# CHONSPQX/modulated-deform-conv

Hardware: AMD Instinct MI355X
Metric: fwd+bwd GSamples/s, MDCN2d 3x3 C=256 56x56 B=32; %HBM roofline (higher is better)
Workload: dtype f32; 1 GPU; ModulatedDeformConv2d 3x3, C_in=C_out=256, 56x56, deformable_group=1, fp32, B=32 per GPU, forward+backward (BASELINE.json configs[1]); global_batch=32, parallelism=dp1 batch-sharded

## Files before the change

### include/mdconv.h

```cpp
#ifndef MDCONV_H_
#define MDCONV_H_

#include <stddef.h>

#ifdef __cplusplus
extern "C" {
#endif

#define MDCONV_ABI_VERSION 2
#define MDCONV_DESC_V2 0x100

enum { MDCONV_F32 = 0, MDCONV_F16 = 1, MDCONV_F64 = 2, MDCONV_BF16 = 3 };
#define MDCONV_SAMPLING_F32 0x10
#define MDCONV_WGRAD_F32 0x40

enum {
  MDCONV_OK = 0,
  MDCONV_EINVAL = -1,
  MDCONV_ENULL = -2,
  MDCONV_EWORKSPACE = -3,
  MDCONV_ELAUNCH = -4,
  MDCONV_EUNSUPPORTED = -5
};

// ... 32 lines not shown

#define MDCONV_DESC_INIT(nd) { (nd) | MDCONV_DESC_V2, 0, 0, 0, 0, 0, {0, 0, 1}, {0, 0, 1}, {1, 1, 1}, \
                               {0, 0, 0}, {1, 1, 1}, 1, 1, 64, 0, 1, 0, 0, {0, 0, 0, 0, 0} }

int mdconv_abi_version(void);
const char *mdconv_last_error(void);

int mdconv_out_size(const mdconv_desc *d, int axis);

size_t mdconv_workspace_bytes(const mdconv_desc *d, int backward);

int mdconv_set_path(int path);
int mdconv_last_path(void);
enum { MDCONV_KERNELS_DIRECT = 1, MDCONV_KERNELS_F32 = 2, MDCONV_KERNELS_HP = 3, MDCONV_KERNELS_DEPTHWISE = 4 };
int mdconv_last_kernels(void);
int mdconv_planned_kernels(const mdconv_desc *d, int backward);

int mdconv_profile_enable(int on);
int mdconv_profile_read(int which, double *total_ms);
const char *mdconv_profile_name(int which);
void mdconv_profile_reset(void);

int mdconv_set_accumulate(int on);

enum { MDCONV_LAYOUT_NCHW = 0, MDCONV_LAYOUT_CHANNELS_LAST = 1 };
int mdconv_set_input_layout(int layout);
int mdconv_input_layout_supported(const mdconv_desc *d, int layout, int backward);

int mdconv_result_layout_supported(const mdconv_desc *d, int backward);

// ... 198 lines not shown
```

### modulated_deform_conv_amd/_capi.py

```python
import ctypes
import os
import threading

HERE = os.path.dirname(os.path.abspath(__file__))
LIB_PATH = os.environ.get("MDCONV_LIB") or os.path.join(HERE, "libmdconv_hip.so")

F32, F16, F64, BF16 = 0, 1, 2, 3
SAMPLING_F32 = 0x10
WGRAD_F32 = 0x40
PATH_AUTO, PATH_DIRECT, PATH_MFMA, PATH_DEPTHWISE = 0, 1, 2, 3
ABI_VERSION = 2
DESC_V2 = 0x100
FLAG_DETERMINISTIC = 1
FLAG_NO_GRAD_INPUT = 4
FLAG_NO_GRAD_WEIGHT = 8
FLAG_MATH_BF16 = 32
FLAG_OUTPUT_CHANNELS_LAST = 64
FLAG_GRAD_INPUT_CHANNELS_LAST = 128
FLAG_SOFTMAX = 256

EXPORTS = (
    "mdconv_abi_version", "mdconv_last_error", "mdconv_out_size", "mdconv_workspace_bytes",
    "mdconv_set_path", "mdconv_last_path", "mdconv_last_kernels",
    "mdconv_profile_enable", "mdconv_profile_read", "mdconv_profile_reset", "mdconv_profile_name",
    "mdconv_stream_wait_weight_ready", "mdconv_stream_wait_weight_ready_on", "mdconv_set_accumulate", "mdconv_set_input_layout",
    "mdconv_input_layout_supported", "mdconv_deterministic_supported", "mdconv_math_bf16_used",
    "mdconv_result_layout_supported", "mdconv_planned_kernels",
    "mdconv_deform_conv2d_forward", "mdconv_deform_conv2d_backward",
    "mdconv_modulated_deform_conv2d_forward", "mdconv_modulated_deform_conv2d_backward",
    "mdconv_deform_conv3d_forward", "mdconv_deform_conv3d_backward",
    "mdconv_modulated_deform_conv3d_forward", "mdconv_modulated_deform_conv3d_backward",
    "mdconv_dcnv3_out_size", "mdconv_dcnv3_workspace_bytes", "mdconv_dcnv3_forward", "mdconv_dcnv3_backward",
    "mdconv_msda_value_len", "mdconv_msda_workspace_bytes", "mdconv_msda_forward", "mdconv_msda_backward",
    "mdconv_dcnv4_out_size", "mdconv_dcnv4_offset_mask_len", "mdconv_dcnv4_workspace_bytes", "mdconv_dcnv4_forward",
    "mdconv_dcnv4_backward",
    "mdconv_fda_value_len", "mdconv_fda_loc_attn_len", "mdconv_fda_workspace_bytes", "mdconv_fda_forward", "mdconv_fda_backward",
    "mdconv_droi_workspace_bytes", "mdconv_droi_forward", "mdconv_droi_backward",
    "mdconv_msda3d_value_len", "mdconv_msda3d_workspace_bytes", "mdconv_msda3d_forward", "mdconv_msda3d_backward",
)

EXPORTS_DAGG = ("mdconv_dagg_feature_len", "mdconv_dagg_workspace_bytes", "mdconv_dagg_forward", "mdconv_dagg_backward")
EXPORTS_MSDAP = ("mdconv_msdap_value_len", "mdconv_msdap_points_len", "mdconv_msdap_workspace_bytes", "mdconv_msdap_forward",
                 "mdconv_msdap_backward")
EXPORTS_FDAP = ("mdconv_fdap_value_len", "mdconv_fdap_loc_attn_len", "mdconv_fdap_workspace_bytes", "mdconv_fdap_forward",
                "mdconv_fdap_backward")
EXPORTS_AFDA = ("mdconv_afda_value_len", "mdconv_afda_offs_attn_len", "mdconv_afda_workspace_bytes", "mdconv_afda_forward",
                "mdconv_afda_backward")

SAMP_QUERIES = {"dcnv3": ("out_size",), "msda": ("value_len",), "dcnv4": ("out_size", "offset_mask_len"),
                "fda": ("value_len", "loc_attn_len"), "droi": (), "msda3d": ("value_len",), "dagg": ("feature_len",),
                "msdap": ("value_len", "points_len"), "fdap": ("value_len", "loc_attn_len"),
                "afda": ("value_len", "offs_attn_len")}

# ... 113 lines not shown
        L.mdconv_last_kernels.restype = ctypes.c_int
        L.mdconv_input_layout_supported.argtypes = [ctypes.c_void_p, ctypes.c_int, ctypes.c_int]
        L.mdconv_deterministic_supported.restype = ctypes.c_int
        L.mdconv_deterministic_supported.argtypes = [ctypes.c_void_p, ctypes.c_int]
        has_math_query = hasattr(L, "mdconv_math_bf16_used")
        if has_math_query:
            L.mdconv_math_bf16_used.argtypes = [ctypes.c_void_p, ctypes.c_int]
        has_layout_query = hasattr(L, "mdconv_result_layout_supported")
        if has_layout_query:
            L.mdconv_result_layout_supported.argtypes = [ctypes.c_void_p, ctypes.c_int]
        has_plan_query = hasattr(L, "mdconv_planned_kernels")
        if has_plan_query:
            L.mdconv_planned_kernels.argtypes = [ctypes.c_void_p, ctypes.c_int]
        missing = (() if has_math_query else ("mdconv_math_bf16_used",)) + (() if has_layout_query else ("mdconv_result_layout_supported",))
        missing += () if has_plan_query else ("mdconv_planned_kernels",)
        missing += tuple(n for n in EXPORTS + EXPORTS_DAGG + EXPORTS_MSDAP + EXPORTS_FDAP + EXPORTS_AFDA
                         if n.startswith(tuple("mdconv_%s_" % op for op in SAMP_QUERIES)) and not hasattr(L, n))
        for name in EXPORTS[11:] + EXPORTS_DAGG + EXPORTS_MSDAP + EXPORTS_FDAP + EXPORTS_AFDA:
            if name not in missing:
                getattr(L, name).restype = ctypes.c_int
        for op, queries in SAMP_QUERIES.items():
            if not hasattr(L, "mdconv_%s_workspace_bytes" % op):
                continue
            ws = getattr(L, "mdconv_%s_workspace_bytes" % op)
            ws.restype, ws.argtypes = ctypes.c_size_t, [ctypes.c_void_p, ctypes.c_int]
            for q in queries:
                getattr(L, "mdconv_%s_%s" % (op, q)).argtypes = [ctypes.c_void_p] + ([ctypes.c_int] if q == "out_size" else [])
        if L.mdconv_abi_version() != ABI_VERSION:
            raise ImportError("libmdconv_hip.so ABI version mismatch")
        _lib = L
# ... 25 lines not shown
    prev = lib().mdconv_set_path(names[path] if isinstance(path, str) else int(path))
    return {v: k for k, v in names.items()}[prev]


def last_path():
    return {0: "none", PATH_DIRECT: "direct", PATH_MFMA: "mfma", PATH_DEPTHWISE: "depthwise"}[lib().mdconv_last_path()]


def last_kernels():
    return KERNELS[lib().mdconv_last_kernels()]


KERNELS = {0: "none", 1: "direct", 2: "f32", 3: "hp", 4: "depthwise"}


def planned_kernels(desc, backward):
    return KERNELS[lib().mdconv_planned_kernels(ctypes.byref(desc), int(bool(backward)))]


PROFILE_SLOTS = 5


_modes = threading.local()


def accumulate_mode():
    return getattr(_modes, "accumulate", 1)


class overwrite_grads:
# ... 156 lines not shown
```

### modulated_deform_conv_amd/csrc/mdconv_api.hip

```cpp
#include <stdarg.h>
#include <stdio.h>
#include <stdlib.h>
#include <string.h>

#include <atomic>
#include <iterator>
#include <map>
#include <mutex>
#include <utility>

#include "mdconv_common.hpp"
#include "dw_plan.hpp"
#include "hp_plan.hpp"
#include "mfma_plan.hpp"
#include "samp_api.hpp"

namespace mdconv {

static thread_local char g_err[512] = "";
static thread_local int g_last_path = 0;
static thread_local int g_last_kernels = 0;
static thread_local int g_accumulate = 1;
static thread_local int g_input_layout = 0;
static std::mutex g_wready_mu;
struct WReady { hipEvent_t ev; unsigned long long tick; };
static std::map<std::pair<int, hipStream_t>, WReady> g_wready;
static std::map<int, hipEvent_t> g_wready_latest;
static unsigned long long g_wready_tick = 0;
constexpr size_t kWReadyMax = 64;
static std::atomic<int> g_path{-1};

void set_error(const char *fmt, ...) {
  va_list ap;
  va_start(ap, fmt);
  vsnprintf(g_err, sizeof(g_err), fmt, ap);
  va_end(ap);
// ... 335 lines not shown

static int refuse(const CallPlan &cp, const Geom &g, int dt, int path, bool backward) {
  if (cp.refused == REFUSE_CHANNELS_LAST)
    set_error("channels-last input is only supported by the native 16-bit kernels with C_in a multiple of 32");
  else if (cp.refused == REFUSE_PATH_MFMA)
    set_error("MDCONV_PATH=mfma but this shape/dtype is not supported by the MFMA kernels");
  else if (cp.refused == REFUSE_RESULT_LAYOUT)
    set_layout_refusal(cp, backward);
  else if (cp.refused == REFUSE_PATH_DEPTHWISE)
    set_error("MDCONV_PATH=depthwise but the depthwise kernels do not take this call: %s", cp.dw_reason);
  else
    set_det_refusal(g, dt, path);
  return MDCONV_EUNSUPPORTED;
}

static int run_forward(const mdconv_desc *d, int nd, int modulated, Tensors t, void *ws,
                       size_t ws_bytes, void *stream) {
  g_err[0] = 0;
  Geom g;
  int rc = fill_geom(d, &g);
  if (rc) return rc;
  if (g.nd != nd || (d->modulated != 0) != (modulated != 0)) {
    set_error("descriptor (ndim=%d, modulated=%d) does not match this entry point", g.nd,
              d->modulated);
    return MDCONV_EINVAL;
  }
  Modes md;
  if ((rc = call_modes(d, &md))) return rc;
  if ((rc = require(t.input, "input")) || (rc = require(t.weight, "weight")) ||
      (rc = require(t.offset, "offset")) || (rc = require(t.output, "output")))
    return rc;
  if (modulated && (rc = require(t.mask, "mask"))) return rc;
  if (g.with_bias && (rc = require(t.bias, "bias"))) return rc;
// ... 36 lines not shown
      if (cp.route == ROUTE_F32_SAMP32) return samp32_forward(g, dt, cp.s32, t, ws, s);
      return mfma_forward(g, dt, cp.f32, t, ws, s);
    default:
      g_last_path = MDCONV_PATH_DIRECT;
      g_last_kernels = MDCONV_KERNELS_DIRECT;
      note_direct_fallback(g, dt, false, path);
      if (cp.route != ROUTE_DIRECT_SAMP32) return direct_forward(g, dt, t, s);
      if ((rc = check_ws(ws, ws_bytes, cp.bytes))) return rc;
      return samp32_forward(g, dt, cp.s32, t, ws, s);
  }
}

static int run_backward(const mdconv_desc *d, int nd, int modulated, Tensors t, void *ws,
                        size_t ws_bytes, void *stream) {
  g_err[0] = 0;
  Geom g;
  int rc = fill_geom(d, &g);
  if (rc) return rc;
  if (g.nd != nd || (d->modulated != 0) != (modulated != 0)) {
    set_error("descriptor (ndim=%d, modulated=%d) does not match this entry point", g.nd,
              d->modulated);
    return MDCONV_EINVAL;
  }
  Modes md;
  if ((rc = call_modes(d, &md))) return rc;
  const Skip skip = md.skip;
  if (skip.input) t.grad_input = nullptr;
  if (skip.weight) t.grad_weight = t.grad_bias = nullptr;
  if ((rc = require(t.input, "input")) || (rc = require(t.weight, "weight")) ||
      (rc = require(t.offset, "offset")) || (rc = require(t.grad_output, "grad_output")) ||
// ... 249 lines not shown
int mdconv_stream_wait_weight_ready(void *stream) {
  return wait_weight_ready((hipStream_t)stream, false, nullptr);
}

int mdconv_stream_wait_weight_ready_on(void *stream, void *producer_stream) {
  return wait_weight_ready((hipStream_t)stream, true, (hipStream_t)producer_stream);
}

int mdconv_set_path(int path) {
  const int prev = current_path();
  if (path >= MDCONV_PATH_AUTO && path <= MDCONV_PATH_DEPTHWISE) g_path.store(path);
  return prev;
}
int mdconv_last_path(void) { return g_last_path; }
int mdconv_last_kernels(void) { return g_last_kernels; }

int mdconv_deform_conv2d_forward(const mdconv_desc *d, const void *input, const void *weight,
                                 const void *bias, const void *offset, void *output,
                                 void *workspace, size_t workspace_bytes, void *stream) {
  Tensors t = {};
  t.input = input; t.weight = weight; t.bias = bias; t.offset = offset; t.output = output;
  return run_forward(d, 2, 0, t, workspace, workspace_bytes, stream);
}

int mdconv_deform_conv2d_backward(const mdconv_desc *d, const void *input, const void *weight,
                                  const void *bias, const void *offset, void *grad_input,
                                  void *grad_weight, void *grad_bias, void *grad_offset,
                                  const void *grad_output, void *workspace,
                                  size_t workspace_bytes, void *stream) {
  Tensors t = {};
// ... 76 lines not shown
```

### modulated_deform_conv_amd/csrc/mdconv_common.hpp

```cpp
#pragma once
#include <hip/hip_runtime.h>
#include <hip/hip_fp16.h>
#include <stdint.h>
#include <functional>

#include "../../include/mdconv.h"

namespace mdconv {

#define MDCONV_EPS 1.192092896e-07F

struct Geom {
  int nd, B, C, O, G, DG, K;
  int in_sz[3], out_sz[3], ksz[3], stride[3], pad[3], dil[3];
  int S_i, S_o;
  int Cg, Og, Cdg;
  int N;
  int load_eps;
  int atom_eps;
  int range_gate;
  int with_bias;
  int modulated;
  int acc_data, acc_w;
  int in_cl;
  int cm_pad, cm_real, C_caller;
  int det;
};
__host__ __device__ __forceinline__ int caller_channel(const Geom &g, int c) {
  if (g.cm_pad == 0) return c < g.C ? c : -1;
  const int q = c / g.cm_pad, r = c - q * g.cm_pad;
  return (q < g.DG && r < g.cm_real) ? q * g.cm_real + r : -1;
}
__host__ __device__ __forceinline__ int caller_channels(const Geom &g) { return g.cm_pad ? g.C_caller : g.C; }

template <typename T> struct Acc { using type = float; };
template <> struct Acc<double> { using type = double; };

__device__ __forceinline__ float ld(const float *p) { return *p; }
__device__ __forceinline__ double ld(const double *p) { return *p; }
__device__ __forceinline__ float ld(const __half *p) { return __half2float(*p); }
__device__ __forceinline__ void st(float *p, float v) { *p = v; }
__device__ __forceinline__ void st(double *p, double v) { *p = v; }
__device__ __forceinline__ void st(__half *p, float v) { *p = __float2half(v); }
struct bf16_t { unsigned short bits; };
__device__ __forceinline__ float bf16_bits_to_float(unsigned short b) { return __uint_as_float((unsigned)b << 16); }
__device__ __forceinline__ unsigned short float_to_bf16_bits(float v) {
  const unsigned u = __float_as_uint(v);
  if ((u & 0x7fffffffu) > 0x7f800000u) return (unsigned short)((u >> 16) | 0x40u);
// ... 345 lines not shown
```

### modulated_deform_conv_amd/csrc/mfma_bwd_data.hip

```cpp
#include "mfma_kernels.hpp"
#include "mfma_tile.hpp"
#include <algorithm>
#include <map>
#include <mutex>
#include <stdio.h>
#include <stdlib.h>

namespace mdconv {

namespace {

int grid_for(int64_t total) {
  int64_t b = (total + 255) / 256;
  return (int)(b > 8192 ? 8192 : (b < 1 ? 1 : b));
}

__device__ __forceinline__ void pack_wq_items(const Geom &g, int ochunks, int cblks, const float *__restrict__ w,
                                              float *__restrict__ wq, int64_t first, int64_t step) {
  const int64_t total = (int64_t)g.K * ochunks * cblks * 2 * 64;
  for (int64_t i = first; i < total; i += step) {
    int64_t r = i;
    const int lane = (int)(r & 63); r >>= 6;
    const int q = (int)(r & 1); r >>= 1;
    const int cblk = (int)(r % cblks); r /= cblks;
// ... 28 lines not shown
    pack_wq_items(g, ochunks, cblks, w, wq, (int64_t)bid * 256 + threadIdx.x, (int64_t)nb_pack * 256);
    return;
  }
  bid -= nb_pack;
  if (bid < nb_zero) {
    for (int64_t i = (int64_t)bid * 256 + threadIdx.x; i < cnt_n; i += (int64_t)nb_zero * 256) cnt[i] = 0;
    return;
  }
  bid -= nb_zero;
  const int qx = bid % qtiles, cy = (bid / qtiles) % ctiles, b = bid / (qtiles * ctiles);
  nchw_to_nhwc_tile(t, g.C, g.S_i, x, xt, b, cy * 32, qx * 32);
}



template <int ND, bool MOD, int WAVES_C, int QPQ, bool CL>
__global__ __launch_bounds__(256, 2) void mfma_bwd_data_kernel(
    Geom g, BwdDims bd, const float *__restrict__ input, const float *__restrict__ gout,
    const float *__restrict__ wq, const float *__restrict__ offset, const float *__restrict__ mask,
    float *__restrict__ gcol, float *__restrict__ grad_offset, float *__restrict__ grad_mask,
    float *__restrict__ ga, float *__restrict__ bias_part, int *__restrict__ cnt,
    int *__restrict__ table, const float *__restrict__ xt, int ntiles, int n_full, int n_tail, int tpw) {
  constexpr int NC = 1 << ND, NP = NC / 2;
  constexpr int MB = 2;
  constexpr int WAVES_P = 4 / WAVES_C;
  constexpr int BNP = 32 * WAVES_P;
  constexpr int RB = ND == 2 ? 8 : 4;
  constexpr int NBATCH = MB * 16 / RB;
  constexpr int HS = NBATCH / 2, CPS = NC / HS;
  constexpr int kOob = 0x7ffffff0;
  extern __shared__ __attribute__((aligned(16))) float smem[];
  const int T_o = bd.ochunks;
  const int gpitch = T_o * 16 + 4;
  float *Gs = smem;
  float *red = smem + BNP * gpitch;
  const int kTapGroup = bd.tap_group;

  const int tid = threadIdx.x, lane = tid & 63, kh = lane >> 5;
  const int wave = __builtin_amdgcn_readfirstlane(tid >> 6);
  const int wc = wave / WAVES_P, wp = wave % WAVES_P;

  int u0, u1;
  if ((int)blockIdx.x < n_full) {
    u0 = xcd_remap(blockIdx.x, n_full) * g.K * tpw;
    u1 = u0 + g.K * tpw;
// ... 717 lines not shown
  }
  return n;
}

size_t bwd_data_lds_bytes(const Geom &g, const BwdDims &bd) {
  const int bnp = 32 * (4 / bd.waves_c);
  const int passes = bd.cblks_q / (2 * bd.waves_c);
  const size_t red = (size_t)bd.red_floats;
  const size_t cl = bd.cl_drain ? (size_t)4 * 32 * 64 + (size_t)4 * 32 * (2 * (1 << g.nd) + 4) : 0;
  return ((size_t)bnp * (bd.ochunks * 16 + 4) + red + cl) * sizeof(float);
}

int mfma_bwd_data_f32(const Geom &g, const BwdDims &bd, const Tensors &t, const float *wq,
                      float *gcol, float *ga, float *bias_part, int *cnt, int *table,
                      const float *xt, hipStream_t stream) {
#define LAUNCH_BD_(ND, MOD, WC, QPQ, CL)                                                            \
  do {                                                                                          \
    const int bnp = 32 * (4 / WC);                                                              \
    const int ntiles = (g.N + bnp - 1) / bnp;                                                   \
    const size_t lds = bwd_data_lds_bytes(g, bd);                                               \
     \
     \
     \
     \
    static std::once_flag attr_once;                                                            \
    static hipError_t attr_err = hipSuccess;                                                    \
    std::call_once(attr_once, [] {                                                              \
      attr_err = hipFuncSetAttribute((const void *)mfma_bwd_data_kernel<ND, MOD, WC, QPQ, CL>,  \
                                     hipFuncAttributeMaxDynamicSharedMemorySize, (int)kBwdDataLdsCap); \
    });                                                                                         \
    if (attr_err != hipSuccess) { set_error("hipFuncSetAttribute: %s", hipGetErrorString(attr_err)); return MDCONV_ELAUNCH; } \
     \
     \
    int occ_q = 0;                                                                              \
    {                                                                                           \
      static std::mutex occ_mu;                                                                 \
      static std::map<size_t, int> occ_by_lds;                                                  \
      std::lock_guard<std::mutex> lock(occ_mu);                                                 \
      auto it = occ_by_lds.find(lds);                                                           \
      if (it == occ_by_lds.end()) {                                                             \
        int nq = 0;                                                                             \
        (void)hipOccupancyMaxActiveBlocksPerMultiprocessor(                                     \
            &nq, (const void *)mfma_bwd_data_kernel<ND, MOD, WC, QPQ, CL>, 256, lds);           \
        (void)hipGetLastError();                                                                \
        it = occ_by_lds.emplace(lds, nq > 0 ? nq : (lds * 2 <= 160 * 1024 ? 2 : 1)).first;      \
      }                                                                                         \
      occ_q = it->second;                                                                       \
    }                                                                                           \
    const int slots = num_cus() * occ_q;                                                        \
    const int tpw = 2;                        \
    const int n_full = ntiles / (slots * tpw) * slots;                                          \
    static const bool debug_plan = getenv("MDCONV_DEBUG_PLAN") != nullptr;                      \
    if (debug_plan)                                                                             \
      fprintf(stderr, "[mdconv] GEMM-1 plan: %d tiles, %zu B LDS, %d resident per CU\n", ntiles, lds, occ_q); \
    const int n_tail = (int)std::min<int64_t>((int64_t)(ntiles - n_full * tpw) * g.K, slots);   \
    hipLaunchKernelGGL((mfma_bwd_data_kernel<ND, MOD, WC, QPQ, CL>), dim3(n_full + n_tail), \
                       dim3(256), lds, stream,                                                  \
                       g, bd, (const float *)t.input, (const float *)t.grad_output, wq,         \
                       (const float *)t.offset, (const float *)t.mask, gcol,                    \
                       (float *)t.grad_offset, (float *)t.grad_mask, ga, bias_part, cnt, table, xt,        \
                       ntiles, n_full, n_tail, tpw);                                            \
  } while (0)
                                                \
#define LAUNCH_BD(ND, MOD, WC, QPQ)                                                             \
  do {                                                                                          \
    if (xt != nullptr && bd.cl_drain) LAUNCH_BD_(ND, MOD, WC, QPQ, true);                       \
    else LAUNCH_BD_(ND, MOD, WC, QPQ, false);                                                   \
  } while (0)
#define LAUNCH_BD2(ND, MOD)                                                                     \
  do {                                                                                          \
    const int nbatch = ND == 2 ? 4 : 8, nquads = bd.ochunks / 4;                                \
                   \
    const int qpq = (ND == 2 && g.G == 1 && nquads % nbatch == 0 && nquads / nbatch <= 2) ? nquads / nbatch : 0; \
    if (bd.waves_c == 4) {                                                                      \
      if (ND == 2 && qpq == 1) LAUNCH_BD(ND, MOD, 4, (ND == 2 ? 1 : 0));                        \
      else if (ND == 2 && qpq == 2) LAUNCH_BD(ND, MOD, 4, (ND == 2 ? 2 : 0));                   \
      else LAUNCH_BD(ND, MOD, 4, 0);                                                            \
    } else if (bd.waves_c == 2) LAUNCH_BD(ND, MOD, 2, 0);                                       \
    else LAUNCH_BD(ND, MOD, 1, 0);                                                              \
  } while (0)
  if (g.nd == 2) { if (g.modulated) LAUNCH_BD2(2, true); else LAUNCH_BD2(2, false); }
  else { if (g.modulated) LAUNCH_BD2(3, true); else LAUNCH_BD2(3, false); }
#undef LAUNCH_BD2
#undef LAUNCH_BD
#undef LAUNCH_BD_
  return check_launch("mfma_bwd_data");
}

int csr_zero_f32(const Geom &g, const BwdDims &bd, int *cnt, hipStream_t stream) {
  const int64_t cnt_n = (int64_t)g.B * g.DG * bd.S_e;
  hipLaunchKernelGGL(zero_int_kernel, dim3(grid_for(cnt_n)), dim3(256), 0, stream, cnt, cnt_n);
  return check_launch("zero_cnt");
}

int csr_build_f32(const Geom &g, const BwdDims &bd, const Tensors &t, int *cnt, int *rowptr,
                  void *entries, hipStream_t stream) {
  const int64_t samples = (int64_t)g.B * g.DG * g.K * g.S_o;
  int rc;
// ... 15 lines not shown
```

### modulated_deform_conv_amd/csrc/mfma_fwd.hip

```cpp
#include "mfma_kernels.hpp"

#include <stdio.h>
#include <stdlib.h>
#include <string.h>

#include "mfma_tile.hpp"

namespace mdconv {

namespace {


template <int ND, bool MOD, int BM, int BN, int WM, int WN, bool PADK>
__global__ __launch_bounds__(256) void mfma_fwd_kernel(Geom g, PackDims pd,
                                                       const float *__restrict__ input,
                                                       const float *__restrict__ wp,
                                                       const float *__restrict__ bias,
                                                       const float *__restrict__ offset,
                                                       const float *__restrict__ mask,
                                                       float *__restrict__ output, int ntm, int ntn,
                                                       int full_tiles, int tail_ways, int tail_hi,
                                                       float *__restrict__ part) {
  constexpr int BK = kBK;
  constexpr int NC = 1 << ND;
  constexpr int NP = NC / 2;
  constexpr int MB = WM / 32, NB = WN / 32;
  constexpr int WAVES_N = BN / WN;
  constexpr int KSUBS = 256 / BN;
  constexpr int CPT = BK / KSUBS;
  static_assert((BM / WM) * (BN / WN) == 4, "4 waves per workgroup");
  static_assert(BK == 16 && CPT >= 1 && BN <= 256 && MB * 2 * 1024 <= 4096, "tile shape");

  __shared__ __attribute__((aligned(16))) float Bs[2 * BK * BN];

  const int grp = blockIdx.y;
  int tile, tap_lo = 0, tap_hi = g.K, tail_slot = -1;
  if ((int)blockIdx.x < full_tiles) {
    tile = xcd_remap(blockIdx.x, full_tiles);
  } else {
    tail_slot = blockIdx.x - full_tiles;
    const int hi_slots = tail_hi * (tail_ways + 1);
    int ti, way, wt;
    if (tail_slot < hi_slots) {
      wt = tail_ways + 1;
      ti = tail_slot / wt;
      way = tail_slot - ti * wt;
    } else {
// ... 32 lines not shown
  const rsrc_t r_wp = make_rsrc(wp + (size_t)grp * T * (slab_bytes / 4), (size_t)T * slab_bytes);
  const int a_voff = (((o0 + wm0) / 32) * 2 * 64 + lane) * 16;
  const int img_voff = (b_g * g.C + grp * g.Cg + ksub * CPT) * g.S_i * 4;

  f32x16 acc[MB][NB];
#pragma unroll
  for (int i = 0; i < MB; ++i)
#pragma unroll
    for (int k = 0; k < NB; ++k)
#pragma unroll
      for (int r = 0; r < 16; ++r) acc[i][k][r] = 0.f;

  int voff[NP];
  float wgt[NC];
  float2 rg0[CPT][NP], rg1[CPT][NP];
  float wc0[NC], wc1[NC];
  int cur_tap = -1, cur_dg = -1;
  typedef unsigned long long lanemask_t;
  lanemask_t bad[NC], bad0[NC], bad1[NC];
#pragma unroll
  for (int ci = 0; ci < NC; ++ci) bad[ci] = bad0[ci] = bad1[ci] = 0ull;

  auto issue = [&](float2 (&rg)[CPT][NP], float (&wc)[NC], lanemask_t (&bd)[NC], int tap, int c0) {
    const int dg = g.DG == 1 ? 0 : min(grp * g.Cg + c0, g.C - 1) / g.Cdg;
    if (tap != cur_tap || dg != cur_dg) {
      float delta[ND];
      const int64_t ob = ((int64_t)(b_g * g.DG + dg) * (ND * g.K) + ND * tap) * g.S_o + pix_g;
#pragma unroll
      for (int a = 0; a < ND; ++a) delta[a] = offset[ob + (int64_t)a * g.S_o];
      int tcd[ND];
      tap_coords<ND>(g, tap, tcd);
      TapCoef<ND, float> tc;
      make_tap<ND, float>(g, oc, tcd, delta, false, tc);
      const float m = MOD ? mask[((int64_t)(b_g * g.DG + dg) * g.K + tap) * g.S_o + pix_g] : 1.f;
      int pidx[NP];
      float pwx[NP], pwy[NP];
      make_pairs<ND, float>(g, tc, m, pidx, pwx, pwy);
      bool prx[NP], pry[NP];
      make_pairs_read<ND, float>(g, tc, prx, pry);
// ... 3 lines not shown
        wgt[2 * pi] = pwx[pi];
        wgt[2 * pi + 1] = pwy[pi];
        bad[2 * pi] = __ballot(pry[pi] && !prx[pi]);
        bad[2 * pi + 1] = __ballot(prx[pi] && !pry[pi]);
      }
      cur_tap = tap;
      cur_dg = dg;
    }
    const int soff = c0 * g.S_i * 4;
#pragma unroll
    for (int i = 0; i < CPT; ++i)
#pragma unroll
      for (int pi = 0; pi < NP; ++pi) {
        rg[i][pi] = buf_load2(r_in, voff[pi], soff + i * g.S_i * 4);
      }
#pragma unroll
    for (int ci = 0; ci < NC; ++ci) { wc[ci] = wgt[ci]; bd[ci] = bad[ci]; }
  };
  auto commit = [&](const float2 (&rgl)[CPT][NP], const float (&wc)[NC], const lanemask_t (&bd)[NC], int c0, float *Bb) {
    lanemask_t any_bad = 0ull;
#pragma unroll
    for (int ci = 0; ci < NC; ++ci) any_bad |= bd[ci];
    float2 rg[CPT][NP];
#pragma unroll
    for (int i = 0; i < CPT; ++i)
#pragma unroll
      for (int pi = 0; pi < NP; ++pi) rg[i][pi] = rgl[i][pi];
    if (any_bad != 0ull) {
#pragma unroll
      for (int i = 0; i < CPT; ++i)
#pragma unroll
        for (int pi = 0; pi < NP; ++pi) {
          asm("v_cndmask_b32_e64 %0, %1, 0, %2" : "=v"(rg[i][pi].x) : "v"(rgl[i][pi].x), "s"(bd[2 * pi]));
          asm("v_cndmask_b32_e64 %0, %1, 0, %2" : "=v"(rg[i][pi].y) : "v"(rgl[i][pi].y), "s"(bd[2 * pi + 1]));
// ... 34 lines not shown
        for (int n = 0; n < NB; ++n) b[n] = Bb[(8 * q + s) * BN + n * 32];
#pragma unroll
        for (int i = 0; i < MB; ++i) {
          const float a = s == 0 ? ra[i][q].x : (s == 1 ? ra[i][q].y : (s == 2 ? ra[i][q].z : ra[i][q].w));
#pragma unroll
          for (int n = 0; n < NB; ++n)
            acc[i][n] = __builtin_amdgcn_mfma_f32_32x32x2f32(a, b[n], acc[i][n], 0, 0, 0);
        }
      }
  };

  float4 ra0[MB][2], ra1[MB][2];
  const int a_last = (T - 1) * slab_bytes;
  int a_soff = tap_lo * cchunks * slab_bytes;
  load_a(ra0, a_soff);
  issue(rg0, wc0, bad0, tap_lo, 0);
  issue(rg1, wc1, bad1, tap_lo, BK);
  for (int tap = tap_lo; tap < tap_hi; ++tap) {
    for (int c0 = 0; c0 < pd.Cgp; c0 += 2 * BK) {
      const bool wrap = c0 + 2 * BK >= pd.Cgp;
      const int ntap = wrap ? min(tap + 1, g.K - 1) : tap;
      const int nc0 = wrap ? 0 : c0 + 2 * BK;
      commit(rg0, wc0, bad0, c0, Bs);
      __syncthreads();
      load_a(ra1, a_soff + slab_bytes);
      issue(rg0, wc0, bad0, ntap, nc0);
      __builtin_amdgcn_sched_barrier(0);
      mma(ra0, Bs);
      commit(rg1, wc1, bad1, c0 + BK, Bs + BK * BN);
      __syncthreads();
      a_soff += 2 * slab_bytes;
      load_a(ra0, min(a_soff, a_last));
      issue(rg1, wc1, bad1, ntap, nc0 + BK);
      __builtin_amdgcn_sched_barrier(0);
      mma(ra1, Bs + BK * BN);
    }
  }

  if (tail_slot >= 0) {
    float *dst = part + (size_t)tail_slot * (BM * BN) + wn0 + (lane & 31);
#pragma unroll
    for (int q = 0; q < NB; ++q)
#pragma unroll
      for (int mb = 0; mb < MB; ++mb)
#pragma unroll
        for (int r = 0; r < 16; ++r)
          dst[(wm0 + mb * 32 + (r & 3) + 8 * (r >> 2) + 4 * kh) * BN + q * 32] = acc[mb][q][r];
    return;
// ... 83 lines not shown
int fwd_tail_reduce_launch(int BM, int BN, const Geom &g, const float *part, const float *bias, float *output, int ntm,
                           int tail_tiles, int full_tiles, int ways, int n_hi, hipStream_t stream) {
  if (tail_tiles <= 0) return MDCONV_OK;
#define FWD_TAIL_RED(M, N)                                                                                        \
  hipLaunchKernelGGL((fwd_tail_reduce_kernel<M, N>), dim3(tail_tiles, kTailSlices), dim3(256), 0, stream, g, part, bias, \
                     output, ntm, full_tiles, ways, n_hi)
  if (BM == 256 && BN == 32) FWD_TAIL_RED(256, 32);
  else if (BM == 128 && BN == 64) FWD_TAIL_RED(128, 64);
  else if (BM == 64 && BN == 128) FWD_TAIL_RED(64, 128);
  else if (BM == 64 && BN == 64) FWD_TAIL_RED(64, 64);
  else { set_error("fwd_tail_reduce: no instance for a %d x %d tile", BM, BN); return MDCONV_ELAUNCH; }
#undef FWD_TAIL_RED
  return check_launch("fwd_tail_reduce");
}

namespace {
template <int ND, bool MOD, int BM, int BN, int WM, int WN, bool PADK>
int fwd_tile_slots() {
  static int slots = 0;
  if (!slots) {
    int n = 0;
    (void)hipOccupancyMaxActiveBlocksPerMultiprocessor(
        &n, reinterpret_cast<const void *>(&mfma_fwd_kernel<ND, MOD, BM, BN, WM, WN, PADK>), 256, 0);
    (void)hipGetLastError();
    slots = device_cus() * (n > 0 ? (n < kTailMaxPerCu ? n : kTailMaxPerCu) : 3);
  }
  return slots;
}

template <int ND, bool MOD, int BM, int BN, int WM, int WN, bool PADK>
int launch_fwd_tile_k(const Geom &g, const PackDims &pd, const Tensors &t, const float *wp, float *part,
                      hipStream_t stream) {
  const int ntm = (g.Og + BM - 1) / BM;
  const int ntn = (g.N + BN - 1) / BN;
  int full_tiles, ways, n_hi;
  fwd_tail_plan(g, ntm * ntn, part ? fwd_tile_slots<ND, MOD, BM, BN, WM, WN, PADK>() : 0, &full_tiles, &ways, &n_hi);
  const int tail_tiles = ntm * ntn - full_tiles;
  static const bool debug_plan = getenv("MDCONV_DEBUG_PLAN") != nullptr;
  if (debug_plan)
    fprintf(stderr, "[mdconv] forward plan: %d x %d tile, %d tiles, slots %d, full %d, tail %d x %d tap ranges (%d of them x %d)\n", BM, BN,
            ntm * ntn, part ? fwd_tile_slots<ND, MOD, BM, BN, WM, WN, PADK>() : 0, full_tiles, tail_tiles, ways, n_hi, ways + 1);
  dim3 grid(full_tiles + tail_tiles * ways + n_hi, g.G);
  hipLaunchKernelGGL((mfma_fwd_kernel<ND, MOD, BM, BN, WM, WN, PADK>), grid, dim3(256), 0, stream,
                     g, pd, (const float *)t.input, wp, (const float *)t.bias,
                     (const float *)t.offset, (const float *)t.mask, (float *)t.output, ntm, ntn,
                     full_tiles, ways, n_hi, part);
  int rc = check_launch("mfma_fwd");
  if (rc || tail_tiles == 0) return rc;
  return fwd_tail_reduce_launch(BM, BN, g, part, (const float *)t.bias, (float *)t.output, ntm, tail_tiles, full_tiles, ways,
                                n_hi, stream);
}

template <int ND, bool MOD, int BM, int BN, int WM, int WN>
int launch_fwd_tile(const Geom &g, const PackDims &pd, const Tensors &t, const float *wp, float *part,
                    hipStream_t stream) {
  if (g.Cg % (2 * kBK)) return launch_fwd_tile_k<ND, MOD, BM, BN, WM, WN, true>(g, pd, t, wp, part, stream);
  return launch_fwd_tile_k<ND, MOD, BM, BN, WM, WN, false>(g, pd, t, wp, part, stream);
}

template <int ND, bool MOD>
int launch_fwd(const Geom &g, const PackDims &pd, const Tensors &t, const float *wp, float *part,
               hipStream_t stream) {
  if (pd.BM == 256) return launch_fwd_tile<ND, MOD, 256, 32, 64, 32>(g, pd, t, wp, part, stream);
  if (pd.BM == 128) return launch_fwd_tile<ND, MOD, 128, 64, 64, 32>(g, pd, t, wp, part, stream);
  return launch_fwd_tile<ND, MOD, 64, 128, 64, 32>(g, pd, t, wp, part, stream);
}

}


// ... 15 lines not shown
```

### modulated_deform_conv_amd/csrc/mfma_kernels.hpp

```cpp
#pragma once
#include "mdconv_common.hpp"

namespace mdconv {

bool mfma_supported(const Geom &g, int dtype, bool backward);
size_t mfma_workspace_bytes(const Geom &g, int dtype, bool backward);

int record_weight_ready(hipStream_t stream);

hipStream_t fork_side_stream(hipStream_t stream);
int join_side_stream(hipStream_t stream);

int zero_bytes(void *p, size_t bytes, hipStream_t stream);

void profile_mark(int which, bool begin, hipStream_t stream, const char *name = nullptr);

}
```

### modulated_deform_conv_amd/csrc/mfma_tile.hpp

```cpp
#pragma once
#include "mdconv_common.hpp"

namespace mdconv {

typedef float f32x16 __attribute__((ext_vector_type(16)));

constexpr int kBK = 16;

struct PackDims {
  int Cgp;
  int Ogp;
  int BM;
};

inline PackDims pack_dims(const Geom &g) {
  PackDims pd;
  pd.BM = g.Og > 128 ? 256 : (g.Og > 64 ? 128 : 64);
  pd.Cgp = (g.Cg + 2 * kBK - 1) / (2 * kBK) * (2 * kBK);
  pd.Ogp = (g.Og + pd.BM - 1) / pd.BM * pd.BM;
  return pd;
}

__device__ __forceinline__ int xcd_remap(int bid, int n) {
  const int q = n >> 3, r = n & 7;
// ... 63 lines not shown
#pragma unroll
  for (int r = ty; r < 32; r += 8)
    if (q0 + r < S) dst[(size_t)r * C + tx] = t[tx][r];
}
#endif

int pack_weights_f32(const Geom &g, const PackDims &pd, const float *weight, float *wp, float *wq,
                     hipStream_t stream);
size_t fwd_tail_bytes(const Geom &g);
constexpr int kTailMaxPerCu = 5;
void fwd_tail_plan(const Geom &g, int tiles, int slots, int *full_tiles, int *ways, int *n_hi);
int fwd_tail_reduce_launch(int BM, int BN, const Geom &g, const float *part, const float *bias, float *output, int ntm,
                           int tail_tiles, int full_tiles, int ways, int n_hi, hipStream_t stream);
int mfma_forward_f32(const Geom &g, const PackDims &pd, const Tensors &t, const float *wp, float *part,
                     hipStream_t stream);
bool fwd_channels_last(const Geom &g);
size_t fwd_cl_bytes(const Geom &g);
int mfma_forward_cl_f32(const Geom &g, const PackDims &pd, const Tensors &t, const float *wp, float *part,
                        float *xt, hipStream_t stream);
int mfma_bwd_weight_f32(const Geom &g, const BwdDims &bd, const Tensors &t, const float *ga,
                        const int *table, float *part, const float *bias_part, const float *xt,
                        hipStream_t stream);
int mfma_bwd_weight_cl_launch(const Geom &g, const BwdDims &bd, const float *xt, const float *ga,
                              const int *table, float *part, hipStream_t stream);
int mfma_bwd_weight_cl_occupancy(int nd, bool padn, int wtile);
int mfma_bwd_weight_occupancy(int nd, bool padn, int wtile);
int device_cus();
bool bwd_channels_last(const Geom &g);
int nchw_to_nhwc_f32(const Geom &g, const float *x, float *xt, hipStream_t stream);
int pack_wq_f32(const Geom &g, const BwdDims &bd, const float *weight, float *wq, hipStream_t stream);
// ... 23 lines not shown
```

Baseline: 73.11 GSamples/s.

## Specialize forward and bwd-data MFMA kernels for compile-time canonical 3x3 geometry

Adds a geometry policy template parameter that, for 2-D modulated 3x3 stride-1 pad-1 single-group convolutions, overrides the runtime Geom fields with compile-time constants. The compiler can then fold index arithmetic and branches on kernel size, groups and deformable groups in the forward and backward-data kernels. The forward kernel also drops one set of double-buffered weight/mask state registers by snapshotting state only at tap or deformable-group boundaries, which lowers register pressure. The cost is extra template instantiations and a runtime dispatch check, with an env var to turn it off.

```diff
diff --git a/include/mdconv.h b/include/mdconv.h
--- a/include/mdconv.h
+++ b/include/mdconv.h
@@ -70,6 +70,9 @@
 int mdconv_last_path(void);
 enum { MDCONV_KERNELS_DIRECT = 1, MDCONV_KERNELS_F32 = 2, MDCONV_KERNELS_HP = 3, MDCONV_KERNELS_DEPTHWISE = 4 };
 int mdconv_last_kernels(void);
+enum { MDCONV_GEOMETRY_RUNTIME = 0, MDCONV_GEOMETRY_CANON3X3 = 1 };
+int mdconv_last_geometry(void);
+int mdconv_geometry_is_canonical(const mdconv_desc *d);
 int mdconv_planned_kernels(const mdconv_desc *d, int backward);
 
 int mdconv_profile_enable(int on);
diff --git a/modulated_deform_conv_amd/_capi.py b/modulated_deform_conv_amd/_capi.py
--- a/modulated_deform_conv_amd/_capi.py
+++ b/modulated_deform_conv_amd/_capi.py
@@ -37,6 +37,7 @@
     "mdconv_fda_value_len", "mdconv_fda_loc_attn_len", "mdconv_fda_workspace_bytes", "mdconv_fda_forward", "mdconv_fda_backward",
     "mdconv_droi_workspace_bytes", "mdconv_droi_forward", "mdconv_droi_backward",
     "mdconv_msda3d_value_len", "mdconv_msda3d_workspace_bytes", "mdconv_msda3d_forward", "mdconv_msda3d_backward",
+    "mdconv_last_geometry", "mdconv_geometry_is_canonical",
 )
 
 EXPORTS_DAGG = ("mdconv_dagg_feature_len", "mdconv_dagg_workspace_bytes", "mdconv_dagg_forward", "mdconv_dagg_backward")
@@ -180,6 +181,7 @@
             L.mdconv_planned_kernels.argtypes = [ctypes.c_void_p, ctypes.c_int]
         missing = (() if has_math_query else ("mdconv_math_bf16_used",)) + (() if has_layout_query else ("mdconv_result_layout_supported",))
         missing += () if has_plan_query else ("mdconv_planned_kernels",)
+        missing += tuple(n for n in ("mdconv_last_geometry", "mdconv_geometry_is_canonical") if not hasattr(L, n))
         missing += tuple(n for n in EXPORTS + EXPORTS_DAGG + EXPORTS_MSDAP + EXPORTS_FDAP + EXPORTS_AFDA
                          if n.startswith(tuple("mdconv_%s_" % op for op in SAMP_QUERIES)) and not hasattr(L, n))
         for name in EXPORTS[11:] + EXPORTS_DAGG + EXPORTS_MSDAP + EXPORTS_FDAP + EXPORTS_AFDA:
@@ -235,6 +237,11 @@
 KERNELS = {0: "none", 1: "direct", 2: "f32", 3: "hp", 4: "depthwise"}
 
 
+def last_geometry():
+    L = lib()
+    return "canon3x3" if hasattr(L, "mdconv_last_geometry") and L.mdconv_last_geometry() == 1 else "runtime"
+
+
 def planned_kernels(desc, backward):
     return KERNELS[lib().mdconv_planned_kernels(ctypes.byref(desc), int(bool(backward)))]
 
diff --git a/modulated_deform_conv_amd/csrc/mdconv_api.hip b/modulated_deform_conv_amd/csrc/mdconv_api.hip
--- a/modulated_deform_conv_amd/csrc/mdconv_api.hip
+++ b/modulated_deform_conv_amd/csrc/mdconv_api.hip
@@ -20,6 +20,7 @@
 static thread_local char g_err[512] = "";
 static thread_local int g_last_path = 0;
 static thread_local int g_last_kernels = 0;
+static thread_local int g_last_geometry = 0;
 static thread_local int g_accumulate = 1;
 static thread_local int g_input_layout = 0;
 static std::mutex g_wready_mu;
@@ -385,9 +386,12 @@
   return MDCONV_EUNSUPPORTED;
 }
 
+void note_geometry_variant(int v) { g_last_geometry = v; }
+
 static int run_forward(const mdconv_desc *d, int nd, int modulated, Tensors t, void *ws,
                        size_t ws_bytes, void *stream) {
   g_err[0] = 0;
+  g_last_geometry = 0;
   Geom g;
   int rc = fill_geom(d, &g);
   if (rc) return rc;
@@ -454,6 +458,7 @@
 static int run_backward(const mdconv_desc *d, int nd, int modulated, Tensors t, void *ws,
                         size_t ws_bytes, void *stream) {
   g_err[0] = 0;
+  g_last_geometry = 0;
   Geom g;
   int rc = fill_geom(d, &g);
   if (rc) return rc;
@@ -733,6 +738,11 @@
 }
 int mdconv_last_path(void) { return g_last_path; }
 int mdconv_last_kernels(void) { return g_last_kernels; }
+int mdconv_last_geometry(void) { return g_last_geometry; }
+int mdconv_geometry_is_canonical(const mdconv_desc *d) {
+  Geom g;
+  return fill_geom(d, &g) == MDCONV_OK && geom_is_canon3x3(g) ? 1 : 0;
+}
 
 int mdconv_deform_conv2d_forward(const mdconv_desc *d, const void *input, const void *weight,
                                  const void *bias, const void *offset, void *output,
diff --git a/modulated_deform_conv_amd/csrc/mdconv_common.hpp b/modulated_deform_conv_amd/csrc/mdconv_common.hpp
--- a/modulated_deform_conv_amd/csrc/mdconv_common.hpp
+++ b/modulated_deform_conv_amd/csrc/mdconv_common.hpp
@@ -32,6 +32,44 @@
   return (q < g.DG && r < g.cm_real) ? q * g.cm_real + r : -1;
 }
 __host__ __device__ __forceinline__ int caller_channels(const Geom &g) { return g.cm_pad ? g.C_caller : g.C; }
+
+struct GeomRuntime {
+  static constexpr bool kFixed = false;
+  __device__ __forceinline__ static const Geom &view(const Geom &g) { return g; }
+};
+struct GeomCanon3x3 {
+  static constexpr bool kFixed = true;
+  __device__ __forceinline__ static Geom view(const Geom &g) {
+    Geom v = g;
+    v.nd = 2;
+    v.G = 1;
+    v.DG = 1;
+    v.K = 9;
+    v.Cg = v.Cdg = g.C;
+    v.Og = g.O;
+#pragma unroll
+    for (int a = 0; a < 2; ++a) {
+      v.ksz[a] = 3;
+      v.stride[a] = 1;
+      v.pad[a] = 1;
+      v.dil[a] = 1;
+      v.out_sz[a] = g.in_sz[a];
+    }
+    v.S_o = g.S_i;
+    v.modulated = 1;
+    v.load_eps = 0;
+    v.atom_eps = 1;
+    v.range_gate = 1;
+    return v;
+  }
+};
+inline bool geom_is_canon3x3(const Geom &g) {
+  if (g.nd != 2 || !g.modulated || g.G != 1 || g.DG != 1 || g.K != 9) return false;
+  for (int a = 0; a < 2; ++a)
+    if (g.ksz[a] != 3 || g.stride[a] != 1 || g.pad[a] != 1 || g.dil[a] != 1 || g.out_sz[a] != g.in_sz[a]) return false;
+  return g.S_o == g.S_i && g.Cg == g.C && g.Cdg == g.C && g.Og == g.O && g.load_eps == 0 && g.atom_eps == 1 &&
+         g.range_gate == 1;
+}
 
 template <typename T> struct Acc { using type = float; };
 template <> struct Acc<double> { using type = double; };
diff --git a/modulated_deform_conv_amd/csrc/mfma_bwd_data.hip b/modulated_deform_conv_amd/csrc/mfma_bwd_data.hip
--- a/modulated_deform_conv_amd/csrc/mfma_bwd_data.hip
+++ b/modulated_deform_conv_amd/csrc/mfma_bwd_data.hip
@@ -5,6 +5,7 @@
 #include <mutex>
 #include <stdio.h>
 #include <stdlib.h>
+#include <type_traits>
 
 namespace mdconv {
 
@@ -66,9 +67,10 @@
 
 
 
-template <int ND, bool MOD, int WAVES_C, int QPQ, bool CL>
+
+template <int ND, bool MOD, int WAVES_C, int QPQ, bool CL, typename GP = GeomRuntime>
 __global__ __launch_bounds__(256, 2) void mfma_bwd_data_kernel(
-    Geom g, BwdDims bd, const float *__restrict__ input, const float *__restrict__ gout,
+    Geom g_arg, BwdDims bd, const float *__restrict__ input, const float *__restrict__ gout,
     const float *__restrict__ wq, const float *__restrict__ offset, const float *__restrict__ mask,
     float *__restrict__ gcol, float *__restrict__ grad_offset, float *__restrict__ grad_mask,
     float *__restrict__ ga, float *__restrict__ bias_part, int *__restrict__ cnt,
@@ -81,6 +83,8 @@
   constexpr int NBATCH = MB * 16 / RB;
   constexpr int HS = NBATCH / 2, CPS = NC / HS;
   constexpr int kOob = 0x7ffffff0;
+  static_assert(!GP::kFixed || (ND == 2 && MOD && QPQ > 0), "the canonical geometry is 2-D, modulated, one conv group");
+  const auto &g = GP::view(g_arg);
   extern __shared__ __attribute__((aligned(16))) float smem[];
   const int T_o = bd.ochunks;
   const int gpitch = T_o * 16 + 4;
@@ -828,7 +832,7 @@
 int mfma_bwd_data_f32(const Geom &g, const BwdDims &bd, const Tensors &t, const float *wq,
                       float *gcol, float *ga, float *bias_part, int *cnt, int *table,
                       const float *xt, hipStream_t stream) {
-#define LAUNCH_BD_(ND, MOD, WC, QPQ, CL)                                                            \
+#define LAUNCH_BD_(ND, MOD, WC, QPQ, CL, GP)                                                          \
   do {                                                                                          \
     const int bnp = 32 * (4 / WC);                                                              \
     const int ntiles = (g.N + bnp - 1) / bnp;                                                   \
@@ -840,7 +844,7 @@
     static std::once_flag attr_once;                                                            \
     static hipError_t attr_err = hipSuccess;                                                    \
     std::call_once(attr_once, [] {                                                              \
-      attr_err = hipFuncSetAttribute((const void *)mfma_bwd_data_kernel<ND, MOD, WC, QPQ, CL>,  \
+      attr_err = hipFuncSetAttribute((const void *)mfma_bwd_data_kernel<ND, MOD, WC, QPQ, CL, GP>,  \
                                      hipFuncAttributeMaxDynamicSharedMemorySize, (int)kBwdDataLdsCap); \
     });                                                                                         \
     if (attr_err != hipSuccess) { set_error("hipFuncSetAttribute: %s", hipGetErrorString(attr_err)); return MDCONV_ELAUNCH; } \
@@ -855,7 +859,7 @@
       if (it == occ_by_lds.end()) {                                                             \
         int nq = 0;                                                                             \
         (void)hipOccupancyMaxActiveBlocksPerMultiprocessor(                                     \
-            &nq, (const void *)mfma_bwd_data_kernel<ND, MOD, WC, QPQ, CL>, 256, lds);           \
+            &nq, (const void *)mfma_bwd_data_kernel<ND, MOD, WC, QPQ, CL, GP>, 256, lds);           \
         (void)hipGetLastError();                                                                \
         it = occ_by_lds.emplace(lds, nq > 0 ? nq : (lds * 2 <= 160 * 1024 ? 2 : 1)).first;      \
       }                                                                                         \
@@ -867,8 +871,12 @@
     static const bool debug_plan = getenv("MDCONV_DEBUG_PLAN") != nullptr;                      \
     if (debug_plan)                                                                             \
       fprintf(stderr, "[mdconv] GEMM-1 plan: %d tiles, %zu B LDS, %d resident per CU\n", ntiles, lds, occ_q); \
+    if (debug_plan)                                                                             \
+      fprintf(stderr, "[mdconv] GEMM-1 instance <%d,%d,%d,%d,%d>, geometry: %s\n", ND, (int)MOD, WC, QPQ, (int)CL, \
+              GP::kFixed ? "canonical 3x3 (compile-time)" : "run-time");                       \
+    note_geometry_variant(GP::kFixed ? 1 : 0);                                                  \
     const int n_tail = (int)std::min<int64_t>((int64_t)(ntiles - n_full * tpw) * g.K, slots);   \
-    hipLaunchKernelGGL((mfma_bwd_data_kernel<ND, MOD, WC, QPQ, CL>), dim3(n_full + n_tail), \
+    hipLaunchKernelGGL((mfma_bwd_data_kernel<ND, MOD, WC, QPQ, CL, GP>), dim3(n_full + n_tail), \
                        dim3(256), lds, stream,                                                  \
                        g, bd, (const float *)t.input, (const float *)t.grad_output, wq,         \
                        (const float *)t.offset, (const float *)t.mask, gcol,                    \
@@ -878,8 +886,20 @@
                                                 \
 #define LAUNCH_BD(ND, MOD, WC, QPQ)                                                             \
   do {                                                                                          \
-    if (xt != nullptr && bd.cl_drain) LAUNCH_BD_(ND, MOD, WC, QPQ, true);                       \
-    else LAUNCH_BD_(ND, MOD, WC, QPQ, false);                                                   \
+    if (xt != nullptr && bd.cl_drain) LAUNCH_BD_(ND, MOD, WC, QPQ, true, GeomRuntime);          \
+    else LAUNCH_BD_(ND, MOD, WC, QPQ, false, GeomRuntime);                                      \
+  } while (0)
+ \
+#define LAUNCH_BD_Q(ND, MOD, WC, QPQ)                                                           \
+  do {                                                                                          \
+     \
+    using GPc = std::conditional<(ND == 2 && MOD && (QPQ) > 0), GeomCanon3x3, GeomRuntime>::type; \
+    if (GPc::kFixed && geom_canon3x3_selected(g)) {                                             \
+      if (xt != nullptr && bd.cl_drain) LAUNCH_BD_(ND, MOD, WC, QPQ, true, GPc);                \
+      else LAUNCH_BD_(ND, MOD, WC, QPQ, false, GPc);                                            \
+    } else {                                                                                    \
+      LAUNCH_BD(ND, MOD, WC, QPQ);                                                              \
+    }                                                                                           \
   } while (0)
 #define LAUNCH_BD2(ND, MOD)                                                                     \
   do {                                                                                          \
@@ -887,8 +907,8 @@
                    \
     const int qpq = (ND == 2 && g.G == 1 && nquads % nbatch == 0 && nquads / nbatch <= 2) ? nquads / nbatch : 0; \
     if (bd.waves_c == 4) {                                                                      \
-      if (ND == 2 && qpq == 1) LAUNCH_BD(ND, MOD, 4, (ND == 2 ? 1 : 0));                        \
-      else if (ND == 2 && qpq == 2) LAUNCH_BD(ND, MOD, 4, (ND == 2 ? 2 : 0));                   \
+      if (ND == 2 && qpq == 1) LAUNCH_BD_Q(ND, MOD, 4, (ND == 2 ? 1 : 0));                      \
+      else if (ND == 2 && qpq == 2) LAUNCH_BD_Q(ND, MOD, 4, (ND == 2 ? 2 : 0));                 \
       else LAUNCH_BD(ND, MOD, 4, 0);                                                            \
     } else if (bd.waves_c == 2) LAUNCH_BD(ND, MOD, 2, 0);                                       \
     else LAUNCH_BD(ND, MOD, 1, 0);                                                              \
@@ -896,6 +916,7 @@
   if (g.nd == 2) { if (g.modulated) LAUNCH_BD2(2, true); else LAUNCH_BD2(2, false); }
   else { if (g.modulated) LAUNCH_BD2(3, true); else LAUNCH_BD2(3, false); }
 #undef LAUNCH_BD2
+#undef LAUNCH_BD_Q
 #undef LAUNCH_BD
 #undef LAUNCH_BD_
   return check_launch("mfma_bwd_data");
diff --git a/modulated_deform_conv_amd/csrc/mfma_fwd.hip b/modulated_deform_conv_amd/csrc/mfma_fwd.hip
--- a/modulated_deform_conv_amd/csrc/mfma_fwd.hip
+++ b/modulated_deform_conv_amd/csrc/mfma_fwd.hip
@@ -11,8 +11,8 @@
 namespace {
 
 
-template <int ND, bool MOD, int BM, int BN, int WM, int WN, bool PADK>
-__global__ __launch_bounds__(256) void mfma_fwd_kernel(Geom g, PackDims pd,
+template <int ND, bool MOD, int BM, int BN, int WM, int WN, bool PADK, typename GP = GeomRuntime>
+__global__ __launch_bounds__(256) void mfma_fwd_kernel(Geom g_arg, PackDims pd,
                                                        const float *__restrict__ input,
                                                        const float *__restrict__ wp,
                                                        const float *__restrict__ bias,
@@ -31,6 +31,9 @@
   static_assert((BM / WM) * (BN / WN) == 4, "4 waves per workgroup");
   static_assert(BK == 16 && CPT >= 1 && BN <= 256 && MB * 2 * 1024 <= 4096, "tile shape");
 
+  static_assert(!GP::kFixed || (ND == 2 && MOD), "the canonical geometry is 2-D and modulated");
+  const auto &g = GP::view(g_arg);
+
   __shared__ __attribute__((aligned(16))) float Bs[2 * BK * BN];
 
   const int grp = blockIdx.y;
@@ -93,15 +96,16 @@
   int voff[NP];
   float wgt[NC];
   float2 rg0[CPT][NP], rg1[CPT][NP];
-  float wc0[NC], wc1[NC];
+  float wcm[NC];
   int cur_tap = -1, cur_dg = -1;
   typedef unsigned long long lanemask_t;
-  lanemask_t bad[NC], bad0[NC], bad1[NC];
-#pragma unroll
-  for (int ci = 0; ci < NC; ++ci) bad[ci] = bad0[ci] = bad1[ci] = 0ull;
-
-  auto issue = [&](float2 (&rg)[CPT][NP], float (&wc)[NC], lanemask_t (&bd)[NC], int tap, int c0) {
-    const int dg = g.DG == 1 ? 0 : min(grp * g.Cg + c0, g.C - 1) / g.Cdg;
+  lanemask_t bad[NC], badc[NC];
+#pragma unroll
+  for (int ci = 0; ci < NC; ++ci) bad[ci] = badc[ci] = 0ull;
+
+  auto dg_of = [&](int c0) { return g.DG == 1 ? 0 : min(grp * g.Cg + c0, g.C - 1) / g.Cdg; };
+  auto issue = [&](float2 (&rg)[CPT][NP], int tap, int c0) {
+    const int dg = dg_of(c0);
     if (tap != cur_tap || dg != cur_dg) {
       float delta[ND];
       const int64_t ob = ((int64_t)(b_g * g.DG + dg) * (ND * g.K) + ND * tap) * g.S_o + pix_g;
@@ -135,10 +139,14 @@
       for (int pi = 0; pi < NP; ++pi) {
         rg[i][pi] = buf_load2(r_in, voff[pi], soff + i * g.S_i * 4);
       }
-#pragma unroll
-    for (int ci = 0; ci < NC; ++ci) { wc[ci] = wgt[ci]; bd[ci] = bad[ci]; }
   };
-  auto commit = [&](const float2 (&rgl)[CPT][NP], const float (&wc)[NC], const lanemask_t (&bd)[NC], int c0, float *Bb) {
+  auto take_state = [&]() {
+#pragma unroll
+    for (int ci = 0; ci < NC; ++ci) { wcm[ci] = wgt[ci]; badc[ci] = bad[ci]; }
+  };
+  auto commit = [&](const float2 (&rgl)[CPT][NP], int c0, float *Bb) {
+    const float (&wc)[NC] = wcm;
+    const lanemask_t (&bd)[NC] = badc;
     lanemask_t any_bad = 0ull;
 #pragma unroll
     for (int ci = 0; ci < NC; ++ci) any_bad |= bd[ci];
@@ -203,24 +211,29 @@
   const int a_last = (T - 1) * slab_bytes;
   int a_soff = tap_lo * cchunks * slab_bytes;
   load_a(ra0, a_soff);
-  issue(rg0, wc0, bad0, tap_lo, 0);
-  issue(rg1, wc1, bad1, tap_lo, BK);
+  issue(rg0, tap_lo, 0);
+  take_state();
+  issue(rg1, tap_lo, BK);
   for (int tap = tap_lo; tap < tap_hi; ++tap) {
     for (int c0 = 0; c0 < pd.Cgp; c0 += 2 * BK) {
-      const bool wrap = c0 + 2 * BK >= pd.Cgp;
+      int c_ahead = c0 + 2 * BK;
+      asm volatile("" : "+s"(c_ahead));
+      const bool wrap = c_ahead >= pd.Cgp;
       const int ntap = wrap ? min(tap + 1, g.K - 1) : tap;
       const int nc0 = wrap ? 0 : c0 + 2 * BK;
-      commit(rg0, wc0, bad0, c0, Bs);
+      commit(rg0, c0, Bs);
+      if (g.DG != 1 && dg_of(c0 + BK) != dg_of(c0)) take_state();
       __syncthreads();
       load_a(ra1, a_soff + slab_bytes);
-      issue(rg0, wc0, bad0, ntap, nc0);
+      issue(rg0, ntap, nc0);
       __builtin_amdgcn_sched_barrier(0);
       mma(ra0, Bs);
-      commit(rg1, wc1, bad1, c0 + BK, Bs + BK * BN);
+      commit(rg1, c0 + BK, Bs + BK * BN);
+      if (wrap || (g.DG != 1 && dg_of(nc0) != dg_of(c0 + BK))) take_state();
       __syncthreads();
       a_soff += 2 * slab_bytes;
       load_a(ra0, min(a_soff, a_last));
-      issue(rg1, wc1, bad1, ntap, nc0 + BK);
+      issue(rg1, ntap, nc0 + BK);
       __builtin_amdgcn_sched_barrier(0);
       mma(ra1, Bs + BK * BN);
     }
@@ -334,34 +347,41 @@
   return check_launch("fwd_tail_reduce");
 }
 
+bool geom_canon3x3_selected(const Geom &g) {
+  static const int on = getenv("MDCONV_GEOM_FIXED") ? atoi(getenv("MDCONV_GEOM_FIXED")) : 1;
+  return on != 0 && geom_is_canon3x3(g);
+}
+
 namespace {
-template <int ND, bool MOD, int BM, int BN, int WM, int WN, bool PADK>
+template <int ND, bool MOD, int BM, int BN, int WM, int WN, bool PADK, typename GP>
 int fwd_tile_slots() {
   static int slots = 0;
   if (!slots) {
     int n = 0;
     (void)hipOccupancyMaxActiveBlocksPerMultiprocessor(
-        &n, reinterpret_cast<const void *>(&mfma_fwd_kernel<ND, MOD, BM, BN, WM, WN, PADK>), 256, 0);
+        &n, reinterpret_cast<const void *>(&mfma_fwd_kernel<ND, MOD, BM, BN, WM, WN, PADK, GP>), 256, 0);
     (void)hipGetLastError();
     slots = device_cus() * (n > 0 ? (n < kTailMaxPerCu ? n : kTailMaxPerCu) : 3);
   }
   return slots;
 }
 
-template <int ND, bool MOD, int BM, int BN, int WM, int WN, bool PADK>
+template <int ND, bool MOD, int BM, int BN, int WM, int WN, bool PADK, typename GP = GeomRuntime>
 int launch_fwd_tile_k(const Geom &g, const PackDims &pd, const Tensors &t, const float *wp, float *part,
                       hipStream_t stream) {
   const int ntm = (g.Og + BM - 1) / BM;
   const int ntn = (g.N + BN - 1) / BN;
   int full_tiles, ways, n_hi;
-  fwd_tail_plan(g, ntm * ntn, part ? fwd_tile_slots<ND, MOD, BM, BN, WM, WN, PADK>() : 0, &full_tiles, &ways, &n_hi);
+  fwd_tail_plan(g, ntm * ntn, part ? fwd_tile_slots<ND, MOD, BM, BN, WM, WN, PADK, GP>() : 0, &full_tiles, &ways, &n_hi);
   const int tail_tiles = ntm * ntn - full_tiles;
   static const bool debug_plan = getenv("MDCONV_DEBUG_PLAN") != nullptr;
+  if (debug_plan) fprintf(stderr, "[mdconv] forward geometry: %s\n", GP::kFixed ? "canonical 3x3 (compile-time)" : "run-time");
+  note_geometry_variant(GP::kFixed ? 1 : 0);
   if (debug_plan)
     fprintf(stderr, "[mdconv] forward plan: %d x %d tile, %d tiles, slots %d, full %d, tail %d x %d tap ranges (%d of them x %d)\n", BM, BN,
-            ntm * ntn, part ? fwd_tile_slots<ND, MOD, BM, BN, WM, WN, PADK>() : 0, full_tiles, tail_tiles, ways, n_hi, ways + 1);
+            ntm * ntn, part ? fwd_tile_slots<ND, MOD, BM, BN, WM, WN, PADK, GP>() : 0, full_tiles, tail_tiles, ways, n_hi, ways + 1);
   dim3 grid(full_tiles + tail_tiles * ways + n_hi, g.G);
-  hipLaunchKernelGGL((mfma_fwd_kernel<ND, MOD, BM, BN, WM, WN, PADK>), grid, dim3(256), 0, stream,
+  hipLaunchKernelGGL((mfma_fwd_kernel<ND, MOD, BM, BN, WM, WN, PADK, GP>), grid, dim3(256), 0, stream,
                      g, pd, (const float *)t.input, wp, (const float *)t.bias,
                      (const float *)t.offset, (const float *)t.mask, (float *)t.output, ntm, ntn,
                      full_tiles, ways, n_hi, part);
@@ -374,6 +394,12 @@
 template <int ND, bool MOD, int BM, int BN, int WM, int WN>
 int launch_fwd_tile(const Geom &g, const PackDims &pd, const Tensors &t, const float *wp, float *part,
                     hipStream_t stream) {
+  if constexpr (ND == 2 && MOD && BM == 256) {
+    if (geom_canon3x3_selected(g)) {
+      if (g.Cg % (2 * kBK)) return launch_fwd_tile_k<ND, MOD, BM, BN, WM, WN, true, GeomCanon3x3>(g, pd, t, wp, part, stream);
+      return launch_fwd_tile_k<ND, MOD, BM, BN, WM, WN, false, GeomCanon3x3>(g, pd, t, wp, part, stream);
+    }
+  }
   if (g.Cg % (2 * kBK)) return launch_fwd_tile_k<ND, MOD, BM, BN, WM, WN, true>(g, pd, t, wp, part, stream);
   return launch_fwd_tile_k<ND, MOD, BM, BN, WM, WN, false>(g, pd, t, wp, part, stream);
 }
diff --git a/modulated_deform_conv_amd/csrc/mfma_kernels.hpp b/modulated_deform_conv_amd/csrc/mfma_kernels.hpp
--- a/modulated_deform_conv_amd/csrc/mfma_kernels.hpp
+++ b/modulated_deform_conv_amd/csrc/mfma_kernels.hpp
@@ -11,6 +11,8 @@
 hipStream_t fork_side_stream(hipStream_t stream);
 int join_side_stream(hipStream_t stream);
 
+void note_geometry_variant(int v);
+
 int zero_bytes(void *p, size_t bytes, hipStream_t stream);
 
 void profile_mark(int which, bool begin, hipStream_t stream, const char *name = nullptr);
diff --git a/modulated_deform_conv_amd/csrc/mfma_tile.hpp b/modulated_deform_conv_amd/csrc/mfma_tile.hpp
--- a/modulated_deform_conv_amd/csrc/mfma_tile.hpp
+++ b/modulated_deform_conv_amd/csrc/mfma_tile.hpp
@@ -101,6 +101,7 @@
                            int tail_tiles, int full_tiles, int ways, int n_hi, hipStream_t stream);
 int mfma_forward_f32(const Geom &g, const PackDims &pd, const Tensors &t, const float *wp, float *part,
                      hipStream_t stream);
+bool geom_canon3x3_selected(const Geom &g);
 bool fwd_channels_last(const Geom &g);
 size_t fwd_cl_bytes(const Geom &g);
 int mfma_forward_cl_f32(const Geom &g, const PackDims &pd, const Tensors &t, const float *wp, float *part,
```

New measurement: 73.88 GSamples/s, median of 6. 1.1% higher.
